# OnurBasci/TransformerBasedNavierStokeSolver

Measured on AMD Instinct MI355X. Metric: ns64_train_samples_per_s, higher is better.
Workload: dtype f32

## Files before the change

transformerbasednavierstokesolver_amd/csrc/pa2d_gemm.hip:

```cpp
#include "pa2d_gemm_common.h"
#include <string.h>


static Pa2dEnv read_env() {
    auto is = [](const char* n, const char* pre) { const char* e = getenv(n); return e && strncmp(e, pre, strlen(pre)) == 0; };
    auto num = [](const char* n, int dflt) { const char* e = getenv(n); return (e && e[0]) ? atoi(e) : dflt; };
    Pa2dEnv v;
    v.conv_halo = is("PA2D_CONV_HALO", "o") ? 0 : (is("PA2D_CONV_HALO", "f") ? 2 : 1);
    v.mc_big_off = is("PA2D_MC_BIG", "o") ? 1 : 0;
    v.kc_bk16 = num("PA2D_KC_BK", 0) == 16 ? 1 : 0;
    v.mc_bk = num("PA2D_MC_BK", 16) == 32 ? 32 : 16;
    v.mc_splits = num("PA2D_MC_SPLITS", 0);
    v.mcb_splits = num("PA2D_MCB_SPLITS", 0);
    v.lin_dw_split = is("PA2D_LIN_DW_SPLIT", "of") ? 0 : 1;
    v.lin_panel = is("PA2D_LIN_PANEL", "of") ? 0 : 1;
    v.lin_rowpanel = is("PA2D_LIN_ROWPANEL", "of") ? 0 : 1;
    v.lin_small_split = is("PA2D_LIN_SMALL_SPLIT", "of") ? 0 : 1;
    v.conv_mfma16 = num("PA2D_CONV_MFMA", 16) == 32 ? 0 : 1;
    v.split_big = num("PA2D_SPLIT_BIG", 1);
    v.slice_map = is("PA2D_SLICE_MAP", "l") ? 0 : 1;
    v.default_engine = is("PA2D_GEMM", "f") ? 0 : (is("PA2D_GEMM", "b") ? 2 : 1);
    return v;
}
static Pa2dEnv g_env = read_env();
const Pa2dEnv& pa2d_env() { return g_env; }
static int kc_bk(bool im2col, int Cin) {
    if (im2col && pa2d_env().kc_bk16) return 16;
    return (!im2col || (Cin % 32) == 0) ? 32 : 16;
}
KCTile kc_tile(int M, int N, bool im2col, int Cin) {
    const int tiles_m = ceil_div(M, 128);
    const long long t128 = (long long)tiles_m * ceil_div(N, 128);
    const long long t12864 = (long long)tiles_m * ceil_div(N, 64);
    const int bk = kc_bk(im2col, Cin);
    if (N > 64 && t128 >= 384) return {128, 128, bk};
    if (t12864 >= 384 || M <= 64) return {128, 64, bk};
    return {64, 64, bk};
}
bool use_split(int engine, int N, bool im2col, int Cin) {
    const int m = engine;
    if (m == 1) return im2col && N > 64 && (Cin % 32) == 0;
    if (m == 2) return N > 64 && (!im2col || (Cin % 32) == 0);
    return false;
}

int launch_kc(const KCParams& p_in, bool im2col, hipStream_t st, hipEvent_t ev0, hipEvent_t ev1) {
    KCParams p = p_in;
    if (!engine_ok(p.engine)) return PA2D_ERR_ARG;
    if (p.M <= 0 || p.N <= 0 || p.K <= 0) return PA2D_OK;
    if (!p.bias2) p.bias_split = 0x7fffffff;
    {
        const unsigned long long ab = ((unsigned long long)(p.M - 1) * p.lda + (im2col ? p.Cin : p.K)) * 4ull;
        const unsigned long long bb = ((unsigned long long)(p.N - 1) * p.ldb + p.K) * 4ull;
        if (ab >= 0xFFFFFFF0ull || bb >= 0xFFFFFFF0ull) return PA2D_ERR_UNSUPPORTED;
        p.a_bytes = (unsigned)ab;
        p.b_bytes = (unsigned)bb;
        const unsigned long long es = p.io_bf16 ? 2ull : 4ull;
        const unsigned long long cb = ((unsigned long long)(p.M - 1) * p.ldc + p.N) * es;
        const unsigned long long rb = p.res ? ((unsigned long long)(p.M - 1) * p.ldres + p.N) * es : 0ull;
        const unsigned long long xb = p.aux ? ((unsigned long long)(p.M - 1) * p.ldaux + p.N) * es : 0ull;
        if (cb >= 0xFFFFFFF0ull || rb >= 0xFFFFFFF0ull || xb >= 0xFFFFFFF0ull) return PA2D_ERR_UNSUPPORTED;
        p.c_bytes = (unsigned)cb; p.res_bytes = (unsigned)rb; p.aux_bytes = (unsigned)xb;
    }
    if ((p.K & 3) || (p.lda & 3) || (p.ldb & 3)) return PA2D_ERR_ARG;
    if (im2col && ((p.Cin & 15) || p.K != (p.taps == 27 ? 27 : 9) * p.Cin)) return PA2D_ERR_UNSUPPORTED;
    if (im2col && (p.epi != 0 || p.res)) return PA2D_ERR_ARG;
    if (ev0 && hipEventRecord(ev0, st) != hipSuccess) return PA2D_ERR_ARG;
    int rc;
    if (!im2col && p.wimg && rowpanel_applies(p)) {
        if (p.wsrc) {
            rc = launch_pack_weight_image(p.wsrc, p.wsn, p.wsk, p.wimg, p.N, p.K, st);
            if (rc) return rc;
        }
        KCParams pp = p;
        pp.M = p.M - p.M % 128;
        rc = launch_kc_rowpanel(pp, p.wimg, st);
        if (!rc && pp.M < p.M) {
            KCParams pt = p_in;
            pt.wimg = nullptr;
            pt.M = p.M - pp.M;
            pt.A = p.A + (size_t)pp.M * p.lda;
            pt.C = p.C + (size_t)pp.M * p.ldc;
            if (p.res) pt.res = p.res + (size_t)pp.M * p.ldres;
            if (p.aux) pt.aux = p.aux + (size_t)pp.M * p.ldaux;
            rc = launch_kc(pt, false, st);
        }
    } else if (panel_applies(p, im2col)) {
        KCParams pp = p;
        pp.M = p.M - p.M % 256;
        rc = launch_kc_panel(pp, st);
        if (!rc && pp.M < p.M) {
            KCParams pt = p_in;
            const size_t ea = p.io_bf16 ? 2 : 4, es = p.io_bf16 ? 2 : 4;
            pt.M = p.M - pp.M;
            pt.A = (const float*)((const char*)p.A + (size_t)pp.M * p.lda * ea);
            pt.C = (float*)((char*)p.C + (size_t)pp.M * p.ldc * es);
            if (p.res) pt.res = (const float*)((const char*)p.res + (size_t)pp.M * p.ldres * es);
            if (p.aux) pt.aux = (float*)((char*)p.aux + (size_t)pp.M * p.ldaux * es);
            rc = launch_kc(pt, false, st);
        }
    } else if (p.io_bf16 || use_split(p.engine, p.N, im2col, p.Cin)) rc = launch_kc_split(p, im2col, st);
    else if (kc_split_small_applies(p, im2col)) rc = launch_kc_split_small(p, st);
    else rc = launch_kc_f32(p, im2col, kc_tile(p.M, p.N, im2col, p.Cin), st);
    if (rc) return rc;
    if (ev1 && hipEventRecord(ev1, st) != hipSuccess) return PA2D_ERR_ARG;
    return PA2D_OK;
}

template <int TAPS>
__global__ void repack_kernel(const float* __restrict__ w0, const float* __restrict__ w1, float* __restrict__ dst,
                              int mode, int N, int K, int C, int Cin, int NK) {
    const long long idx = (long long)blockIdx.x * blockDim.x + threadIdx.x;
    if (mode == 0) {
        if (idx >= (long long)N * K) return;
        const int n = (int)(idx % N), k = (int)(idx / N);
        dst[idx] = w0[(size_t)n * K + k];
    } else if (mode == 1) {
        if (idx >= (long long)NK * C * TAPS * Cin) return;
        const int CH = K;
        const int c16 = (int)(idx % CH);
        const int tap = (int)((idx / CH) % TAPS);
        const int cic = (int)((idx / (TAPS * CH)) % (Cin / CH));
        const int co = (int)(idx / ((long long)Cin * TAPS));
        const int ci = cic * CH + c16;
        const float* src = co < C ? w0 : w1;
        dst[idx] = src[((size_t)(co % C) * Cin + ci) * TAPS + tap];
    } else {
        if (idx >= (long long)NK * C * TAPS * Cin) return;
        const int CH = K;
        const int c16 = (int)(idx % CH);
        const int tap = (int)((idx / CH) % TAPS);
        const int cic = (int)((idx / (TAPS * CH)) % (NK * C / CH));
        const int ci = (int)(idx / ((long long)NK * C * TAPS));
        const int co = cic * CH + c16;
        const float* src = co < C ? w0 : w1;
        dst[idx] = src[((size_t)(co % C) * Cin + ci) * TAPS + (TAPS - 1 - tap)];
    }
}

int launch_repack(const float* w0, const float* w1, float* dst, int mode, int N, int K, int C, int Cin, hipStream_t st,
                  int taps) {
    const int nk = w1 ? 2 : 1;
    const long long count = mode == 0 ? (long long)N * K : (long long)nk * C * taps * Cin;
    const dim3 grid((unsigned)ceil_div_ll(count, 256));
    if (taps == 27)
        hipLaunchKernelGGL(repack_kernel<27>, grid, dim3(256), 0, st, w0, w1, dst, mode, N, K, C, Cin, nk);
    else
        hipLaunchKernelGGL(repack_kernel<9>, grid, dim3(256), 0, st, w0, w1, dst, mode, N, K, C, Cin, nk);
    PA2D_CHECK_LAUNCH();
    return PA2D_OK;
}

static KCParams dense_fwd_params(const void* x, long long ldx, const float* w, long long ldw, const float* bias,
                                 const void* res, long long ldres, void* y, long long ldy, void* pre, long long ldpre, int M,
                                 int N, int K, int act, int engine, bool io_bf16) {
    KCParams p = {};
    p.engine = engine; p.io_bf16 = io_bf16 ? 1 : 0; p.apre = io_bf16 ? 1 : 0;
    p.aux_deriv = (act & PA2D_ACT_SAVE_DERIVATIVE_BIT) ? 1 : 0;
    act &= ~PA2D_ACT_SAVE_DERIVATIVE_BIT;
    p.A = (const float*)x; p.lda = ldx; p.B = w; p.ldb = ldw; p.C = (float*)y; p.ldc = ldy; p.bias = bias;
    p.res = (const float*)res; p.ldres = ldres; p.aux = (float*)pre; p.ldaux = ldpre; p.M = M; p.N = N; p.K = K; p.act = act;
    p.epi = (act != ACT_NONE ? EPI_ACT : 0) | (pre ? EPI_STORE_PRE : 0);
    return p;
}
static KCParams dense_bwd_data_params(const void* dy, long long lddy, const float* wt, const void* pre, long long ldpre,
                                      int act, void* dx, long long lddx, int M, int N, int K, int engine, bool io_bf16) {
// ... 133 lines not shown
```

transformerbasednavierstokesolver_amd/csrc/pa2d_gemm_mc_planes.hip:

```cpp
#include "pa2d_gemm_common.h"
#include "pa2d_bf16_split.h"

struct MCPlanesParams {
    const void* PA; int chA;
    const void* PB; int chB;
    float* slab;
    int Mi, Nj, Mk, chunks_per_split, splits, H, W, Cin;
    unsigned a_bytes, b_bytes;
    int taps;
    long long lda, ldb;
    float* colsum;
};

__device__ __forceinline__ unsigned img_off(int row, int ch) {
    return 256u * row + 16u * (ch ^ (((row & 3) << 2) | ((row >> 2) & 3)));
}

template <int NT, int KS, bool F32SRC = false>
__global__ __launch_bounds__(256, 2) void gemm_mc_planes_kernel(const MCPlanesParams p) {
    constexpr int PIMG = 4096;
    constexpr int STAGE = 2 * NT * KS * PIMG;
    constexpr int NP = 2 * NT * KS;
    __shared__ __attribute__((aligned(16))) unsigned char smem[2 * STAGE];

// ... 69 lines not shown
            bool ok_ = m_ < p.Mk && (KS == 1 || (c_) + (s_row[s] >> 4) < c_end);    \
            int mm_ = m_;                                                                                 \
            if (s_isb[s]) {                                                                               \
                const int n_ = m_ % HW;                                                                   \
                const int y_ = n_ / p.W, x_ = n_ - y_ * p.W;                                              \
                ok_ = ok_ && (unsigned)(y_ + tap_dy) < (unsigned)p.H && (unsigned)(x_ + tap_dx) < (unsigned)p.W; \
                mm_ = m_ + tap_shift;                                                                     \
            }                                                                                             \
            const unsigned rowb_ = (unsigned)mm_ * (unsigned)((s_isb[s] ? p.chB : p.chA) * NT * 64);      \
            rg[s] = s_isb[s] ? __builtin_amdgcn_raw_buffer_load_b128(rb_rsrc, ok_ ? rowb_ + s_goff[s] : OOB_OFF, 0, 0) \
                             : __builtin_amdgcn_raw_buffer_load_b128(ra_rsrc, ok_ ? rowb_ + s_goff[s] : OOB_OFF, 0, 0); \
        }                                                                                                 \
    }
#define MP_STORE(buf_)                                                                                    \
    if constexpr (F32SRC) {                                                                               \
        _Pragma("unroll") for (int ks = 0; ks < KS; ++ks) _Pragma("unroll") for (int op = 0; op < 2; ++op) { \
            const u32x4 u0_ = rg[ks * 4 + op * 2], u1_ = rg[ks * 4 + op * 2 + 1];                         \
            const float4 v0_ = make_float4(__uint_as_float(u0_.x), __uint_as_float(u0_.y), __uint_as_float(u0_.z), __uint_as_float(u0_.w)); \
            const float4 v1_ = make_float4(__uint_as_float(u1_.x), __uint_as_float(u1_.y), __uint_as_float(u1_.z), __uint_as_float(u1_.w)); \
            if (op == 0 && do_cs) {                                                                       \
                cs[0] += v0_.x; cs[1] += v0_.y; cs[2] += v0_.z; cs[3] += v0_.w;                           \
                cs[4] += v1_.x; cs[5] += v1_.y; cs[6] += v1_.z; cs[7] += v1_.w;                           \
            }                                                                                             \
            bf16x4 h0_, m0_, l0_, h1_, m1_, l1_;                                                          \
            split3(v0_, h0_, m0_, l0_);                                                                   \
            split3(v1_, h1_, m1_, l1_);                                                                   \
            unsigned char* d_ = smem + (buf_) * STAGE + flds;                                             \
            *reinterpret_cast<bf16x8*>(d_ + ((op * NT + 0) * KS + ks) * PIMG) = __builtin_shufflevector(h0_, h1_, 0, 1, 2, 3, 4, 5, 6, 7); \
            if (NT == 3) {                                                                                \
                *reinterpret_cast<bf16x8*>(d_ + ((op * NT + 1) * KS + ks) * PIMG) = __builtin_shufflevector(m0_, m1_, 0, 1, 2, 3, 4, 5, 6, 7); \
                *reinterpret_cast<bf16x8*>(d_ + ((op * NT + 2) * KS + ks) * PIMG) = __builtin_shufflevector(l0_, l1_, 0, 1, 2, 3, 4, 5, 6, 7); \
            }                                                                                             \
        }                                                                                                 \
    } else {                                                                                              \
        _Pragma("unroll") for (int s = 0; s < NP; ++s)                                                    \
            *reinterpret_cast<u32x4*>(smem + (buf_) * STAGE + s_lds[s]) = rg[s];                          \
    }
    const bool do_cs = F32SRC && p.colsum != nullptr && tj == 0;

    f32x16 acc[2][2];
#pragma unroll
    for (int i = 0; i < 2; ++i)
#pragma unroll
        for (int j = 0; j < 2; ++j)
#pragma unroll
            for (int r = 0; r < 16; ++r) acc[i][j][r] = 0.f;

    const int g = lane >> 4, q4 = (lane & 15) >> 2, pq = lane & 3;
    unsigned fa[2][2], fb[2][2];
#pragma unroll
    for (int t = 0; t < 2; ++t)
#pragma unroll
        for (int r = 0; r < 2; ++r) {
            const int row = 8 * (g >> 1) + 4 * r + q4;
            const int cha = ((wm * 64 + t * 32) >> 3) + 2 * (g & 1) + (pq >> 1);
            const int chb = ((wn * 64 + t * 32) >> 3) + 2 * (g & 1) + (pq >> 1);
            fa[t][r] = img_off(row, cha) + 8u * (pq & 1);
            fb[t][r] = img_off(row, chb) + 8u * (pq & 1);
        }

    if (c_begin < c_end) {
        MP_LOAD(c_begin)
        MP_STORE(0)
    }
    __syncthreads();
    for (int c = c_begin; c < c_end; c += KS) {
        const int buf = ((c - c_begin) / KS) & 1;
        if (c + KS < c_end) { MP_LOAD(c + KS) }
#pragma unroll
        for (int ks = 0; ks < KS; ++ks) {
        const unsigned char* st = smem + buf * STAGE + ks * PIMG;
        bf16x8 af[2][NT], bf[2][NT];
#pragma unroll
        for (int t = 0; t < 2; ++t)
#pragma unroll
            for (int pl = 0; pl < NT; ++pl) {
                typedef __attribute__((address_space(3))) s16x4 lds_s16x4;
                const s16x4 a0 = __builtin_amdgcn_ds_read_tr16_b64_v4i16((lds_s16x4*)(st + pl * KS * PIMG + fa[t][0]));
                const s16x4 a1 = __builtin_amdgcn_ds_read_tr16_b64_v4i16((lds_s16x4*)(st + pl * KS * PIMG + fa[t][1]));
                const s16x4 b0 = __builtin_amdgcn_ds_read_tr16_b64_v4i16((lds_s16x4*)(st + (NT + pl) * KS * PIMG + fb[t][0]));
                const s16x4 b1 = __builtin_amdgcn_ds_read_tr16_b64_v4i16((lds_s16x4*)(st + (NT + pl) * KS * PIMG + fb[t][1]));
                const s16x8 av = __builtin_shufflevector(a0, a1, 0, 1, 2, 3, 4, 5, 6, 7);
                const s16x8 bv = __builtin_shufflevector(b0, b1, 0, 1, 2, 3, 4, 5, 6, 7);
                af[t][pl] = __builtin_bit_cast(bf16x8, av);
                bf[t][pl] = __builtin_bit_cast(bf16x8, bv);
            }
#pragma unroll
        for (int i = 0; i < 2; ++i)
#pragma unroll
            for (int j = 0; j < 2; ++j) {
                if constexpr (NT == 3) {
                    acc[i][j] = __builtin_amdgcn_mfma_f32_32x32x16_bf16(af[i][1], bf[j][1], acc[i][j], 0, 0, 0);
                    acc[i][j] = __builtin_amdgcn_mfma_f32_32x32x16_bf16(af[i][2], bf[j][0], acc[i][j], 0, 0, 0);
                    acc[i][j] = __builtin_amdgcn_mfma_f32_32x32x16_bf16(af[i][0], bf[j][2], acc[i][j], 0, 0, 0);
                    acc[i][j] = __builtin_amdgcn_mfma_f32_32x32x16_bf16(af[i][1], bf[j][0], acc[i][j], 0, 0, 0);
                    acc[i][j] = __builtin_amdgcn_mfma_f32_32x32x16_bf16(af[i][0], bf[j][1], acc[i][j], 0, 0, 0);
                }
                acc[i][j] = __builtin_amdgcn_mfma_f32_32x32x16_bf16(af[i][0], bf[j][0], acc[i][j], 0, 0, 0);
            }
        }
        if (c + KS < c_end) { MP_STORE(buf ^ 1) }
        __syncthreads();
    }
#undef MP_LOAD
#undef MP_STORE

    if constexpr (F32SRC) {
        if (do_cs) {
            float* sm = reinterpret_cast<float*>(smem);
#pragma unroll
            for (int e = 0; e < 8; ++e) sm[frow * 128 + fc8 * 8 + e] = cs[e];
            __syncthreads();
            if (tid < 128) {
                float t = 0.f;
#pragma unroll
                for (int r = 0; r < 16; ++r) t += sm[r * 128 + tid];
                if (ti * 128 + tid < p.Mi) p.colsum[(size_t)split * p.Mi + ti * 128 + tid] = t;
            }
        }
    }
    float* out = p.slab + (size_t)split * p.Mi * p.Nj;
    const int col0 = tj * 128 + wn * 64 + (lane & 31);
    const int row0 = ti * 128 + wm * 64 + 4 * (lane >> 5);
#pragma unroll
    for (int j = 0; j < 2; ++j)
#pragma unroll
        for (int i = 0; i < 2; ++i)
#pragma unroll
            for (int r = 0; r < 16; ++r) {
                const int row = row0 + i * 32 + (r & 3) + 8 * (r >> 2);
                if (!F32SRC || (row < p.Mi && col0 + j * 32 < p.Nj)) out[(size_t)row * p.Nj + col0 + j * 32] = acc[i][j][r];
            }
}

bool mc_planes_supported(int C, int Cin) { return (C % 64) == 0 && (Cin % 128) == 0; }

int launch_mc_planes(const void* PA, const void* PB, int C, int Cin, int Mk, int H, int W, float* slab,
                     const MCPlan& pl, int NT, hipStream_t st) {
    if (!mc_planes_supported(C, Cin) || !pl.big) return PA2D_ERR_UNSUPPORTED;
    MCPlanesParams p;
    p.PA = PA; p.chA = 2 * C / 32; p.PB = PB; p.chB = Cin / 32; p.slab = slab;
    p.Mi = 2 * C; p.Nj = 9 * Cin; p.Mk = Mk; p.chunks_per_split = pl.chunks_per_split; p.splits = pl.splits;
    p.H = H; p.W = W; p.Cin = Cin; p.taps = 9;
    const unsigned long long ab = (unsigned long long)Mk * p.chA * NT * 64, bb = (unsigned long long)Mk * p.chB * NT * 64;
    if (ab >= 0xFFFFFFF0ull || bb >= 0xFFFFFFF0ull) return PA2D_ERR_UNSUPPORTED;
    p.a_bytes = (unsigned)ab; p.b_bytes = (unsigned)bb;
    const dim3 grid((p.Mi / 128) * (p.Nj / 128) * pl.splits);
    if (NT == 3) hipLaunchKernelGGL((gemm_mc_planes_kernel<3, 1>), grid, dim3(256), 0, st, p);
    else hipLaunchKernelGGL((gemm_mc_planes_kernel<1, 4>), grid, dim3(256), 0, st, p);
    PA2D_CHECK_LAUNCH();
    return PA2D_OK;
}

template <int NT, int KS>
__global__ __launch_bounds__(512, 1) void gemm_mc_planes_big_kernel(const MCPlanesParams p, const int per_xcd) {
    constexpr int PIMG = 8192;
    constexpr int STAGE = 2 * NT * KS * PIMG;
    constexpr int NP = (2 * NT * KS * 512) / 512;
    extern __shared__ __attribute__((aligned(16))) unsigned char smem[];

    const int tid = threadIdx.x, lane = tid & 63, wave = tid >> 6;
    const int tiles_i = (p.Mi + 255) / 256, tiles_j = (p.Nj + 255) / 256;
    const int tiles = tiles_i * tiles_j;
    const int lin = (blockIdx.x & 7) * per_xcd + (blockIdx.x >> 3);
    if ((int)(blockIdx.x >> 3) >= per_xcd || lin >= tiles * p.splits) return;
    const int split = lin / tiles, t_ = lin - split * tiles;
    const int ti = t_ / tiles_j, tj = t_ - ti * tiles_j;
    const int wm = wave >> 2, wn = wave & 3;
    const int total_chunks = (p.Mk + 15) / 16;
    const int c_begin = split * p.chunks_per_split;
    const int c_end = min(total_chunks, c_begin + p.chunks_per_split);
    const int HW = p.taps == 1 ? 1 : p.H * p.W;

    const __amdgpu_buffer_rsrc_t ra_rsrc = __builtin_amdgcn_make_buffer_rsrc(const_cast<void*>(p.PA), 0, p.a_bytes, 0x00020000);
    const __amdgpu_buffer_rsrc_t rb_rsrc = __builtin_amdgcn_make_buffer_rsrc(const_cast<void*>(p.PB), 0, p.b_bytes, 0x00020000);

    const int row16 = tid >> 5, cgrp = (tid & 31) >> 2, piece = tid & 3;
    const bool colok_a = ti * 256 + cgrp * 32 < p.Mi;
    const unsigned goff_a = (unsigned)((((ti * 256) >> 5) + cgrp) * NT * 64 + piece * 16);
    const int jc = tj * 256 + cgrp * 32;
    const int tap = p.taps == 1 ? 4 : jc / p.Cin;
    const bool colok_b = jc < p.Nj;
    const unsigned goff_b = (unsigned)((p.taps == 1 ? (jc >> 5) : ((jc - tap * p.Cin) >> 5)) * NT * 64 + piece * 16);
    const int tap_dy = tap / 3 - 1, tap_dx = tap - (tap / 3) * 3 - 1, tap_shift = tap_dy * p.W + tap_dx;
    const unsigned pitch_a = (unsigned)(p.chA * NT * 64), pitch_b = (unsigned)(p.chB * NT * 64);
    const unsigned lds_off = 512u * row16 + 16u * ((unsigned)(cgrp * 4 + piece) ^ (unsigned)(((row16 & 3) << 2) | ((row16 >> 2) & 3)));
#define MB_LOAD(c_, RG)                                                                                   \
    {                                                                                                     \
        _Pragma("unroll") for (int ks = 0; ks < KS; ++ks) {                                               \
            const int m_ = ((c_) + ks) * 16 + row16;                                                      \
            const bool okr_ = m_ < p.Mk && (c_) + ks < c_end;             \
            bool okb_ = okr_ && colok_b;                                                                  \
            int mm_ = m_;                                                                                 \
            if (p.taps != 1) {       \
                okb_ = okb_ && (unsigned)(ly + tap_dy) < (unsigned)p.H && (unsigned)(lx + tap_dx) < (unsigned)p.W; \
                mm_ = m_ + tap_shift;                                                                     \
                lx += 16;                                                                                 \
                while (lx >= p.W) { lx -= p.W; ++ly; }                                                    \
                while (ly >= p.H) ly -= p.H;                                                              \
            }                                                                                             \
            const unsigned oa_ = (okr_ && colok_a) ? (unsigned)m_ * pitch_a + goff_a : OOB_OFF;           \
            const unsigned ob_ = okb_ ? (unsigned)mm_ * pitch_b + goff_b : OOB_OFF;                       \
            _Pragma("unroll") for (int pl = 0; pl < NT; ++pl) {                                           \
                RG[pl * KS + ks] = __builtin_amdgcn_raw_buffer_load_b128(ra_rsrc, oa_ == OOB_OFF ? OOB_OFF : oa_ + pl * 64u, 0, 0); \
                RG[(NT + pl) * KS + ks] = __builtin_amdgcn_raw_buffer_load_b128(rb_rsrc, ob_ == OOB_OFF ? OOB_OFF : ob_ + pl * 64u, 0, 0); \
            }                                                                                             \
        }                                                                                                 \
    }
#define MB_STORE(buf_, RG)                                                                                \
    {                                                                                                     \
        _Pragma("unroll") for (int s = 0; s < NP; ++s)                                                    \
            *reinterpret_cast<u32x4*>(smem + (buf_) * STAGE + s * PIMG + lds_off) = RG[s];                \
    }
    u32x4 rg0[NP];
    int ly = 0, lx = 0;
    if (p.taps != 1) {
        const int n0 = (c_begin * 16 + row16) % HW;
        ly = n0 / p.W;
        lx = n0 - ly * p.W;
    }

    f32x16 acc[4][2];
#pragma unroll
    for (int i = 0; i < 4; ++i)
#pragma unroll
        for (int j = 0; j < 2; ++j)
#pragma unroll
            for (int r = 0; r < 16; ++r) acc[i][j][r] = 0.f;

    const int g = lane >> 4, q4 = (lane & 15) >> 2, pq = lane & 3;
    unsigned fa[4][2], fb[2][2];
#pragma unroll
    for (int r = 0; r < 2; ++r) {
        const int row = 8 * (g >> 1) + 4 * r + q4;
        const unsigned swz = (unsigned)(((row & 3) << 2) | ((row >> 2) & 3));
#pragma unroll
        for (int t = 0; t < 4; ++t) {
            const int cha = ((wm * 128 + t * 32) >> 3) + 2 * (g & 1) + (pq >> 1);
            fa[t][r] = 512u * row + 16u * ((unsigned)cha ^ swz) + 8u * (pq & 1);
        }
#pragma unroll
        for (int t = 0; t < 2; ++t) {
            const int chb = ((wn * 64 + t * 32) >> 3) + 2 * (g & 1) + (pq >> 1);
            fb[t][r] = 512u * row + 16u * ((unsigned)chb ^ swz) + 8u * (pq & 1);
        }
    }

#define MB_COMPUTE(buf_)                                                                                  \
    _Pragma("unroll") for (int ks = 0; ks < KS; ++ks) {                                                   \
        const unsigned char* st = smem + (buf_) * STAGE + ks * PIMG;                                      \
        bf16x8 af[4][NT], bf[2][NT];                                                                      \
        typedef __attribute__((address_space(3))) s16x4 lds_s16x4;                                        \
        _Pragma("unroll") for (int pl = 0; pl < NT; ++pl) {                                               \
            _Pragma("unroll") for (int t = 0; t < 4; ++t) {                                               \
                const s16x4 a0 = __builtin_amdgcn_ds_read_tr16_b64_v4i16((lds_s16x4*)(st + pl * KS * PIMG + fa[t][0])); \
                const s16x4 a1 = __builtin_amdgcn_ds_read_tr16_b64_v4i16((lds_s16x4*)(st + pl * KS * PIMG + fa[t][1])); \
                af[t][pl] = __builtin_bit_cast(bf16x8, __builtin_shufflevector(a0, a1, 0, 1, 2, 3, 4, 5, 6, 7)); \
            }                                                                                             \
            _Pragma("unroll") for (int t = 0; t < 2; ++t) {                                               \
                const s16x4 b0 = __builtin_amdgcn_ds_read_tr16_b64_v4i16((lds_s16x4*)(st + (NT + pl) * KS * PIMG + fb[t][0])); \
                const s16x4 b1 = __builtin_amdgcn_ds_read_tr16_b64_v4i16((lds_s16x4*)(st + (NT + pl) * KS * PIMG + fb[t][1])); \
                bf[t][pl] = __builtin_bit_cast(bf16x8, __builtin_shufflevector(b0, b1, 0, 1, 2, 3, 4, 5, 6, 7)); \
            }                                                                                             \
        }                                                                                                 \
        _Pragma("unroll") for (int i = 0; i < 4; ++i)                                                     \
            _Pragma("unroll") for (int j = 0; j < 2; ++j) {                                               \
                if constexpr (NT == 3) {                                        \
                    acc[i][j] = __builtin_amdgcn_mfma_f32_32x32x16_bf16(af[i][1], bf[j][1], acc[i][j], 0, 0, 0); \
                    acc[i][j] = __builtin_amdgcn_mfma_f32_32x32x16_bf16(af[i][2], bf[j][0], acc[i][j], 0, 0, 0); \
                    acc[i][j] = __builtin_amdgcn_mfma_f32_32x32x16_bf16(af[i][0], bf[j][2], acc[i][j], 0, 0, 0); \
                    acc[i][j] = __builtin_amdgcn_mfma_f32_32x32x16_bf16(af[i][1], bf[j][0], acc[i][j], 0, 0, 0); \
                    acc[i][j] = __builtin_amdgcn_mfma_f32_32x32x16_bf16(af[i][0], bf[j][1], acc[i][j], 0, 0, 0); \
                }                                                                                         \
                acc[i][j] = __builtin_amdgcn_mfma_f32_32x32x16_bf16(af[i][0], bf[j][0], acc[i][j], 0, 0, 0); \
            }                                                                                             \
    }
    if (c_begin < c_end) {
        MB_LOAD(c_begin, rg0)
        MB_STORE(0, rg0)
        if (c_begin + KS < c_end) MB_LOAD(c_begin + KS, rg0)
    }
    __syncthreads();
    for (int c = c_begin; c < c_end; c += KS) {
        const int buf = ((c - c_begin) / KS) & 1;
        if (c + KS < c_end) {
            MB_STORE(buf ^ 1, rg0)
            if (c + 2 * KS < c_end) MB_LOAD(c + 2 * KS, rg0)
        }
        MB_COMPUTE(buf)
        __syncthreads();
    }
#undef MB_COMPUTE
#undef MB_LOAD
#undef MB_STORE

    float* out = p.slab + (size_t)split * p.Mi * p.Nj;
    const int col0 = tj * 256 + wn * 64 + (lane & 31);
    const int row0 = ti * 256 + wm * 128 + 4 * (lane >> 5);
#pragma unroll
    for (int j = 0; j < 2; ++j) {
        const int col = col0 + j * 32;
        if (col >= p.Nj) continue;
#pragma unroll
        for (int i = 0; i < 4; ++i)
#pragma unroll
            for (int r = 0; r < 16; ++r) {
                const int row = row0 + i * 32 + (r & 3) + 8 * (r >> 2);
                if (row < p.Mi) out[(size_t)row * p.Nj + col] = acc[i][j][r];
            }
    }
}

MCPlan plan_mc_planes_big(int Mi, int Nj, int Mk) {
    MCPlan pl;
    if (Mk < 1) Mk = 1;
    pl.big = 2;
    const int tiles = ceil_div(Mi, 256) * ceil_div(Nj, 256);
    const int total_chunks = ceil_div(Mk, 16);
    int splits = 256 / tiles;
    if (pa2d_env().mcb_splits > 0) splits = pa2d_env().mcb_splits;
    const int max_splits = total_chunks / 8 > 0 ? total_chunks / 8 : 1;
    if (splits > max_splits) splits = max_splits;
    if (splits < 1) splits = 1;
    pl.chunks_per_split = ceil_div(total_chunks, splits);
    pl.splits = ceil_div(total_chunks, pl.chunks_per_split);
    pl.slab_floats = (size_t)pl.splits * Mi * Nj;
    return pl;
}

bool mc_planes_big_applies(int C, int Cin, int Mk) {
    if (pa2d_env().mc_big_off) return false;
    return (C % 16) == 0 && (Cin % 32) == 0 && 2 * C >= 256 && 9 * Cin >= 256 && Mk >= 16 * 8 * 4;
}

int launch_mc_planes_big(const void* PA, const void* PB, int C, int Cin, int Mk, int H, int W, float* slab,
                         const MCPlan& pl, int NT, hipStream_t st) {
    return launch_mc_planes_big_raw(PA, 2 * C, PB, Cin, 9, Mk, H, W, slab, pl, NT, st);
}

int launch_mc_planes_big_raw(const void* PA, int Mi, const void* PB, int Cin, int taps, int Mk, int H, int W, float* slab,
                             const MCPlan& pl, int NT, hipStream_t st) {
    if ((Mi & 31) || (Cin & 31) || (taps != 1 && taps != 9)) return PA2D_ERR_UNSUPPORTED;
    MCPlanesParams p;
    p.PA = PA; p.chA = Mi / 32; p.PB = PB; p.chB = Cin / 32; p.slab = slab;
    p.Mi = Mi; p.Nj = taps * Cin; p.Mk = Mk; p.chunks_per_split = pl.chunks_per_split; p.splits = pl.splits;
    p.H = H; p.W = W; p.Cin = Cin; p.taps = taps;
    const unsigned long long ab = (unsigned long long)Mk * p.chA * NT * 64, bb = (unsigned long long)Mk * p.chB * NT * 64;
    if (ab >= 0xFFFFFFF0ull || bb >= 0xFFFFFFF0ull) return PA2D_ERR_UNSUPPORTED;
    p.a_bytes = (unsigned)ab; p.b_bytes = (unsigned)bb;
    const int wgs = ceil_div(p.Mi, 256) * ceil_div(p.Nj, 256) * pl.splits;
    const int per_xcd = ceil_div(wgs, 8);
    const dim3 grid(per_xcd * 8);
    if (NT == 3) {
        const int smem = 2 * 2 * 3 * 1 * 8192;
        {
            hipError_t e = hipFuncSetAttribute(reinterpret_cast<const void*>(&gemm_mc_planes_big_kernel<3, 1>),
                                               hipFuncAttributeMaxDynamicSharedMemorySize, smem);
            if (e != hipSuccess) return (int)e;
        }
        hipLaunchKernelGGL((gemm_mc_planes_big_kernel<3, 1>), grid, dim3(512), smem, st, p, per_xcd);
    } else {
        const int smem = 2 * 2 * 1 * 4 * 8192;
        {
            hipError_t e = hipFuncSetAttribute(reinterpret_cast<const void*>(&gemm_mc_planes_big_kernel<1, 4>),
                                               hipFuncAttributeMaxDynamicSharedMemorySize, smem);
            if (e != hipSuccess) return (int)e;
        }
        hipLaunchKernelGGL((gemm_mc_planes_big_kernel<1, 4>), grid, dim3(512), smem, st, p, per_xcd);
    }
    PA2D_CHECK_LAUNCH();
    return PA2D_OK;
}

bool mc_f32src_applies(int Mi, int Nj, int Mk, long long lda, long long ldb) {
    return pa2d_env().lin_dw_split && (Mi % 8) == 0 && (Nj % 8) == 0 && Mi > 64 && Nj > 64 && Mk >= 16 * 8 * 16 && (lda % 4) == 0 && (ldb % 4) == 0;
}

int launch_mc_f32src(const float* A, long long lda, int Mi, const float* B, long long ldb, int Nj, int Mk, float* slab,
                     const MCPlan& pl, int NT, float* colsum, hipStream_t st) {
    if (!pl.big) return PA2D_ERR_UNSUPPORTED;
    MCPlanesParams p = {};
    p.PA = A; p.PB = B; p.slab = slab; p.lda = lda; p.ldb = ldb; p.colsum = colsum;
    p.Mi = Mi; p.Nj = Nj; p.Mk = Mk; p.chunks_per_split = pl.chunks_per_split; p.splits = pl.splits;
    p.H = 1; p.W = 1; p.Cin = Nj; p.taps = 1; p.chA = 0; p.chB = 0;
    const unsigned long long ab = ((unsigned long long)(Mk - 1) * lda + Mi) * 4ull, bb = ((unsigned long long)(Mk - 1) * ldb + Nj) * 4ull;
    if (ab >= 0xFFFFFFF0ull || bb >= 0xFFFFFFF0ull) return PA2D_ERR_UNSUPPORTED;
    p.a_bytes = (unsigned)ab; p.b_bytes = (unsigned)bb;
    const dim3 grid(ceil_div(Mi, 128) * ceil_div(Nj, 128) * pl.splits);
    if (NT == 3) hipLaunchKernelGGL((gemm_mc_planes_kernel<3, 1, true>), grid, dim3(256), 0, st, p);
    else hipLaunchKernelGGL((gemm_mc_planes_kernel<1, 4, true>), grid, dim3(256), 0, st, p);
    PA2D_CHECK_LAUNCH();
    return PA2D_OK;
}
```

transformerbasednavierstokesolver_amd/csrc/pa2d_internal.h:

```cpp
#pragma once
#include <hip/hip_runtime.h>
#include <stdint.h>

typedef float f32x16 __attribute__((ext_vector_type(16)));
typedef float f32x4 __attribute__((ext_vector_type(4)));

#define PA2D_OK 0
#define PA2D_ERR_ARG 1001
#define PA2D_ERR_UNSUPPORTED 1002
#define PA2D_ERR_WORKSPACE 1003

#define PA2D_CHECK_LAUNCH()                         \
    do {                                            \
        hipError_t e__ = hipGetLastError();         \
        if (e__ != hipSuccess) return (int)e__;     \
    } while (0)

enum { ACT_NONE = 0, ACT_GELU = 1, ACT_TANH = 2, ACT_SIGMOID = 3, ACT_RELU = 4, ACT_SOFTPLUS = 5,
       ACT_ELU = 6, ACT_SILU = 7 };

__device__ __forceinline__ float normal_cdf(float x, float& e_out) {
#pragma clang fp contract(off)
    const float z = fabsf(x) * 0.70710678118654752440f;
    const float t = __builtin_amdgcn_rcpf(fmaf(0.3275911f, z, 1.0f));
    float poly = fmaf(1.061405429f, t, -1.453152027f);
    poly = fmaf(poly, t, 1.421413741f);
    poly = fmaf(poly, t, -0.284496736f);
    poly = fmaf(poly, t, 0.254829592f);
    const float e = __builtin_amdgcn_exp2f(-z * z * 1.44269504088896340736f);
    e_out = e;
    const float hq = 0.5f * poly * t * e;
    return x < 0.f ? hq : 1.0f - hq;
}
__device__ __forceinline__ float gelu_exact(float x) {
#pragma clang fp contract(off)
    float e;
    return x * normal_cdf(x, e);
}
__device__ __forceinline__ float dgelu_exact(float x) {
#pragma clang fp contract(off)
    float e;
    const float cdf = normal_cdf(x, e);
    return fmaf(x * 0.39894228040143267794f, e, cdf);
}

__device__ __forceinline__ float act_fwd(int id, float x) {
    switch (id) {
        case ACT_GELU: return gelu_exact(x);
        case ACT_TANH: return tanhf(x);
        case ACT_SIGMOID: return 1.0f / (1.0f + expf(-x));
        case ACT_RELU: return x > 0.f ? x : 0.f;
        case ACT_SOFTPLUS: return x > 20.f ? x : log1pf(expf(x));
        case ACT_ELU: return x > 0.f ? x : expm1f(x);
        case ACT_SILU: return x / (1.0f + expf(-x));
        default: return x;
    }
}

__device__ __forceinline__ float act_bwd(int id, float x) {
    switch (id) {
        case ACT_GELU: return dgelu_exact(x);
        case ACT_TANH: { const float t = tanhf(x); return 1.0f - t * t; }
        case ACT_SIGMOID: { const float s = 1.0f / (1.0f + expf(-x)); return s * (1.0f - s); }
        case ACT_RELU: return x > 0.f ? 1.f : 0.f;
        case ACT_SOFTPLUS: return x > 20.f ? 1.f : 1.0f / (1.0f + expf(-x));
        case ACT_ELU: return x > 0.f ? 1.f : expf(x);
        case ACT_SILU: { const float s = 1.0f / (1.0f + expf(-x)); return s * (1.0f + x * (1.0f - s)); }
        default: return 1.f;
    }
}

__device__ __forceinline__ float wave_sum(float v) {
#pragma unroll
    for (int o = 32; o > 0; o >>= 1) v += __shfl_xor(v, o, 64);
    return v;
}
__device__ __forceinline__ float wave_max(float v) {
#pragma unroll
    for (int o = 32; o > 0; o >>= 1) v = fmaxf(v, __shfl_xor(v, o, 64));
    return v;
}

typedef unsigned int u32x4 __attribute__((ext_vector_type(4)));
#define OOB_OFF 0xFFFFFFFFu

__device__ __forceinline__ __amdgpu_buffer_rsrc_t make_rsrc(const float* base, unsigned bytes) {
    return __builtin_amdgcn_make_buffer_rsrc(const_cast<float*>(base), 0, bytes, 0x00020000);
}
__device__ __forceinline__ float4 buf_load4(__amdgpu_buffer_rsrc_t r, unsigned voff) {
    const u32x4 v = __builtin_amdgcn_raw_buffer_load_b128(r, voff, 0, 0);
    return make_float4(__uint_as_float(v.x), __uint_as_float(v.y), __uint_as_float(v.z), __uint_as_float(v.w));
}


__device__ __forceinline__ float buf_load1(__amdgpu_buffer_rsrc_t r, unsigned voff) {
    return __uint_as_float(__builtin_amdgcn_raw_buffer_load_b32(r, voff, 0, 0));
}
__device__ __forceinline__ void buf_store1(__amdgpu_buffer_rsrc_t r, unsigned voff, float v) {
    __builtin_amdgcn_raw_buffer_store_b32(__float_as_uint(v), r, voff, 0, 0);
}

__device__ __forceinline__ float2 buf_load2(__amdgpu_buffer_rsrc_t r, unsigned voff) {
    typedef unsigned int u32x2_ __attribute__((ext_vector_type(2)));
    const u32x2_ v = __builtin_amdgcn_raw_buffer_load_b64(r, voff, 0, 0);
    return make_float2(__uint_as_float(v.x), __uint_as_float(v.y));
}
__device__ __forceinline__ void buf_store4(__amdgpu_buffer_rsrc_t r, unsigned voff, float4 v) {
    u32x4 u = {__float_as_uint(v.x), __float_as_uint(v.y), __float_as_uint(v.z), __float_as_uint(v.w)};
    __builtin_amdgcn_raw_buffer_store_b128(u, r, voff, 0, 0);
}

#define PA2D_ACT_SAVE_DERIVATIVE_BIT 0x100

struct Pa2dEnv {
    int conv_halo;
    int mc_big_off;
    int kc_bk16;
    int mc_bk;
    int mc_splits;
    int mcb_splits;
    int lin_dw_split;
    int lin_panel;
    int conv_mfma16;
    int lin_small_split;
    int lin_rowpanel;
    int split_big;
    int slice_map;
    int default_engine;
};
const Pa2dEnv& pa2d_env();

static inline int pa2d_zero(void* p, size_t bytes, hipStream_t st) {
    if (!p || !bytes) return PA2D_OK;
    return (int)hipMemsetAsync(p, 0, bytes, st);
}
static inline int ceil_div(int a, int b) { return (a + b - 1) / b; }
static inline long long ceil_div_ll(long long a, long long b) { return (a + b - 1) / b; }

struct ReduceSegs { int nseg; long long begin[5]; float* dst[4]; };
int pa2d_launch_reduce_segs(const float* slab, int nslab, long long count, const ReduceSegs& segs, int accumulate,
                            hipStream_t st);

typedef __bf16 bf16_t;
template <typename T> struct Act;
template <> struct Act<float> {
    static constexpr unsigned ES = 4;
    static __device__ __forceinline__ float4 ld4(const float* p) { return *reinterpret_cast<const float4*>(p); }
    static __device__ __forceinline__ void st4(float* p, float4 v) { *reinterpret_cast<float4*>(p) = v; }
    static __device__ __forceinline__ float ld1(const float* p) { return *p; }
    static __device__ __forceinline__ float4 bld4(__amdgpu_buffer_rsrc_t r, unsigned off) { return buf_load4(r, off); }
    static __device__ __forceinline__ float2 bld2(__amdgpu_buffer_rsrc_t r, unsigned off) { return buf_load2(r, off); }
    static __device__ __forceinline__ float bld1(__amdgpu_buffer_rsrc_t r, unsigned off) { return buf_load1(r, off); }
    static __device__ __forceinline__ float bld1s(__amdgpu_buffer_rsrc_t r, unsigned off, unsigned soff) {
        return __uint_as_float(__builtin_amdgcn_raw_buffer_load_b32(r, off, soff, 0));
    }
    static __device__ __forceinline__ void bst4(__amdgpu_buffer_rsrc_t r, unsigned off, float4 v) { buf_store4(r, off, v); }
    static __device__ __forceinline__ void bst1(__amdgpu_buffer_rsrc_t r, unsigned off, float v) { buf_store1(r, off, v); }
};
__device__ __forceinline__ float bf16_bits_to_f32(unsigned short b) { return __uint_as_float((unsigned)b << 16); }
__device__ __forceinline__ unsigned short f32_to_bf16_bits(float x) {
    const bf16_t h = (bf16_t)x;
    return __builtin_bit_cast(unsigned short, h);
}
__device__ __forceinline__ unsigned pack_bf16x2(float lo, float hi) {
    return (unsigned)f32_to_bf16_bits(lo) | ((unsigned)f32_to_bf16_bits(hi) << 16);
}
template <> struct Act<bf16_t> {
    static constexpr unsigned ES = 2;
    static __device__ __forceinline__ float4 unpack4(uint2 q) {
        return make_float4(__uint_as_float(q.x << 16), __uint_as_float(q.x & 0xFFFF0000u), __uint_as_float(q.y << 16),
                           __uint_as_float(q.y & 0xFFFF0000u));
    }
    static __device__ __forceinline__ float4 ld4(const bf16_t* p) { return unpack4(*reinterpret_cast<const uint2*>(p)); }
    static __device__ __forceinline__ void st4(bf16_t* p, float4 v) {
        *reinterpret_cast<uint2*>(p) = make_uint2(pack_bf16x2(v.x, v.y), pack_bf16x2(v.z, v.w));
    }
    static __device__ __forceinline__ float ld1(const bf16_t* p) { return (float)*p; }
    static __device__ __forceinline__ float4 bld4(__amdgpu_buffer_rsrc_t r, unsigned off) {
        typedef unsigned int u32x2_ __attribute__((ext_vector_type(2)));
        const u32x2_ q = __builtin_amdgcn_raw_buffer_load_b64(r, off, 0, 0);
        return unpack4(make_uint2(q.x, q.y));
    }
    static __device__ __forceinline__ float2 bld2(__amdgpu_buffer_rsrc_t r, unsigned off) {
        const unsigned q = __builtin_amdgcn_raw_buffer_load_b32(r, off, 0, 0);
        return make_float2(__uint_as_float(q << 16), __uint_as_float(q & 0xFFFF0000u));
    }
    static __device__ __forceinline__ float bld1(__amdgpu_buffer_rsrc_t r, unsigned off) {
        return bf16_bits_to_f32(__builtin_amdgcn_raw_buffer_load_b16(r, off, 0, 0));
    }
    static __device__ __forceinline__ float bld1s(__amdgpu_buffer_rsrc_t r, unsigned off, unsigned soff) {
        return bf16_bits_to_f32(__builtin_amdgcn_raw_buffer_load_b16(r, off, soff, 0));
    }
    static __device__ __forceinline__ void bst4(__amdgpu_buffer_rsrc_t r, unsigned off, float4 v) {
        typedef unsigned int u32x2_ __attribute__((ext_vector_type(2)));
        const u32x2_ q = {pack_bf16x2(v.x, v.y), pack_bf16x2(v.z, v.w)};
        __builtin_amdgcn_raw_buffer_store_b64(q, r, off, 0, 0);
    }
    static __device__ __forceinline__ void bst1(__amdgpu_buffer_rsrc_t r, unsigned off, float v) {
        __builtin_amdgcn_raw_buffer_store_b16(f32_to_bf16_bits(v), r, off, 0, 0);
    }
};
__device__ __forceinline__ __amdgpu_buffer_rsrc_t make_rsrc_v(const void* base, unsigned bytes) {
    return __builtin_amdgcn_make_buffer_rsrc(const_cast<void*>(base), 0, bytes, 0x00020000);
}

__device__ __forceinline__ bool slice_decode(int xcd_map, int B, int heads, int nchunk, int& b, int& hh, int& chunk, int& bid) {
    const int total = B * heads * nchunk;
    int L;
    if (xcd_map) {
        const int per = (total + 7) >> 3;
        if ((int)(blockIdx.x >> 3) >= per) return false;
        L = (int)(blockIdx.x & 7) * per + (int)(blockIdx.x >> 3);
        if (L >= total) return false;
        hh = L % heads;
        chunk = (L / heads) % nchunk;
        b = L / (heads * nchunk);
    } else {
        L = (int)blockIdx.x;
        if (L >= total) return false;
        chunk = L % nchunk;
        hh = (L / nchunk) % heads;
        b = L / (nchunk * heads);
    }
    bid = (b * heads + hh) * nchunk + chunk;
    return true;
}
static inline int slice_grid(int total) { return ((total + 7) / 8) * 8; }
```

Measured before the change: 68.44.

## Stagger MFMA schedule across wave halves in big multi-chunk planes GEMM

Adds a staggered variant of the big planes GEMM kernel for the NT=3 case, on by default. Waves 4-7 defer most of their MFMAs for each K-step into the next iteration, running them before the next LDS store and global load. The aim is to shift half the workgroup out of phase so LDS reads, global loads and MFMA work overlap instead of every wave bursting in lockstep between barriers. The cost is extra live fragment registers across the barrier, plus sched_barrier hints that limit the compiler's own scheduling.

```diff
diff --git a/transformerbasednavierstokesolver_amd/csrc/pa2d_gemm.hip b/transformerbasednavierstokesolver_amd/csrc/pa2d_gemm.hip
--- a/transformerbasednavierstokesolver_amd/csrc/pa2d_gemm.hip
+++ b/transformerbasednavierstokesolver_amd/csrc/pa2d_gemm.hip
@@ -12,6 +12,7 @@
     v.mc_bk = num("PA2D_MC_BK", 16) == 32 ? 32 : 16;
     v.mc_splits = num("PA2D_MC_SPLITS", 0);
     v.mcb_splits = num("PA2D_MCB_SPLITS", 0);
+    v.mcb_stagger = is("PA2D_MCB_STAGGER", "of") ? 0 : 1;
     v.lin_dw_split = is("PA2D_LIN_DW_SPLIT", "of") ? 0 : 1;
     v.lin_panel = is("PA2D_LIN_PANEL", "of") ? 0 : 1;
     v.lin_rowpanel = is("PA2D_LIN_ROWPANEL", "of") ? 0 : 1;
diff --git a/transformerbasednavierstokesolver_amd/csrc/pa2d_gemm_mc_planes.hip b/transformerbasednavierstokesolver_amd/csrc/pa2d_gemm_mc_planes.hip
--- a/transformerbasednavierstokesolver_amd/csrc/pa2d_gemm_mc_planes.hip
+++ b/transformerbasednavierstokesolver_amd/csrc/pa2d_gemm_mc_planes.hip
@@ -245,8 +245,9 @@
     return PA2D_OK;
 }
 
-template <int NT, int KS>
+template <int NT, int KS, bool STAG = false>
 __global__ __launch_bounds__(512, 1) void gemm_mc_planes_big_kernel(const MCPlanesParams p, const int per_xcd) {
+    static_assert(!STAG || KS == 1, "the staggered schedule defers part of ONE K-step");
     constexpr int PIMG = 8192;
     constexpr int STAGE = 2 * NT * KS * PIMG;
     constexpr int NP = (2 * NT * KS * 512) / 512;
@@ -339,34 +340,38 @@
         }
     }
 
+    typedef __attribute__((address_space(3))) s16x4 lds_s16x4;
+#define MB_READS(st_, AF, BF)                                                                             \
+    _Pragma("unroll") for (int pl = 0; pl < NT; ++pl) {                                                   \
+        _Pragma("unroll") for (int t = 0; t < 4; ++t) {                                                   \
+            const s16x4 a0 = __builtin_amdgcn_ds_read_tr16_b64_v4i16((lds_s16x4*)((st_) + pl * KS * PIMG + fa[t][0])); \
+            const s16x4 a1 = __builtin_amdgcn_ds_read_tr16_b64_v4i16((lds_s16x4*)((st_) + pl * KS * PIMG + fa[t][1])); \
+            AF[t][pl] = __builtin_bit_cast(bf16x8, __builtin_shufflevector(a0, a1, 0, 1, 2, 3, 4, 5, 6, 7)); \
+        }                                                                                                 \
+        _Pragma("unroll") for (int t = 0; t < 2; ++t) {                                                   \
+            const s16x4 b0 = __builtin_amdgcn_ds_read_tr16_b64_v4i16((lds_s16x4*)((st_) + (NT + pl) * KS * PIMG + fb[t][0])); \
+            const s16x4 b1 = __builtin_amdgcn_ds_read_tr16_b64_v4i16((lds_s16x4*)((st_) + (NT + pl) * KS * PIMG + fb[t][1])); \
+            BF[t][pl] = __builtin_bit_cast(bf16x8, __builtin_shufflevector(b0, b1, 0, 1, 2, 3, 4, 5, 6, 7)); \
+        }                                                                                                 \
+    }
+#define MB_MFMAS(T0, T1, AF, BF)                                                                          \
+    _Pragma("unroll") for (int t = (T0); t < (T1); ++t) {                                                 \
+        const int i = t >> 1, j = t & 1;                                                                  \
+        if constexpr (NT == 3) {                                                \
+            acc[i][j] = __builtin_amdgcn_mfma_f32_32x32x16_bf16(AF[i][1], BF[j][1], acc[i][j], 0, 0, 0);  \
+            acc[i][j] = __builtin_amdgcn_mfma_f32_32x32x16_bf16(AF[i][2], BF[j][0], acc[i][j], 0, 0, 0);  \
+            acc[i][j] = __builtin_amdgcn_mfma_f32_32x32x16_bf16(AF[i][0], BF[j][2], acc[i][j], 0, 0, 0);  \
+            acc[i][j] = __builtin_amdgcn_mfma_f32_32x32x16_bf16(AF[i][1], BF[j][0], acc[i][j], 0, 0, 0);  \
+            acc[i][j] = __builtin_amdgcn_mfma_f32_32x32x16_bf16(AF[i][0], BF[j][1], acc[i][j], 0, 0, 0);  \
+        }                                                                                                 \
+        acc[i][j] = __builtin_amdgcn_mfma_f32_32x32x16_bf16(AF[i][0], BF[j][0], acc[i][j], 0, 0, 0);      \
+    }
 #define MB_COMPUTE(buf_)                                                                                  \
     _Pragma("unroll") for (int ks = 0; ks < KS; ++ks) {                                                   \
         const unsigned char* st = smem + (buf_) * STAGE + ks * PIMG;                                      \
         bf16x8 af[4][NT], bf[2][NT];                                                                      \
-        typedef __attribute__((address_space(3))) s16x4 lds_s16x4;                                        \
-        _Pragma("unroll") for (int pl = 0; pl < NT; ++pl) {                                               \
-            _Pragma("unroll") for (int t = 0; t < 4; ++t) {                                               \
-                const s16x4 a0 = __builtin_amdgcn_ds_read_tr16_b64_v4i16((lds_s16x4*)(st + pl * KS * PIMG + fa[t][0])); \
-                const s16x4 a1 = __builtin_amdgcn_ds_read_tr16_b64_v4i16((lds_s16x4*)(st + pl * KS * PIMG + fa[t][1])); \
-                af[t][pl] = __builtin_bit_cast(bf16x8, __builtin_shufflevector(a0, a1, 0, 1, 2, 3, 4, 5, 6, 7)); \
-            }                                                                                             \
-            _Pragma("unroll") for (int t = 0; t < 2; ++t) {                                               \
-                const s16x4 b0 = __builtin_amdgcn_ds_read_tr16_b64_v4i16((lds_s16x4*)(st + (NT + pl) * KS * PIMG + fb[t][0])); \
-                const s16x4 b1 = __builtin_amdgcn_ds_read_tr16_b64_v4i16((lds_s16x4*)(st + (NT + pl) * KS * PIMG + fb[t][1])); \
-                bf[t][pl] = __builtin_bit_cast(bf16x8, __builtin_shufflevector(b0, b1, 0, 1, 2, 3, 4, 5, 6, 7)); \
-            }                                                                                             \
-        }                                                                                                 \
-        _Pragma("unroll") for (int i = 0; i < 4; ++i)                                                     \
-            _Pragma("unroll") for (int j = 0; j < 2; ++j) {                                               \
-                if constexpr (NT == 3) {                                        \
-                    acc[i][j] = __builtin_amdgcn_mfma_f32_32x32x16_bf16(af[i][1], bf[j][1], acc[i][j], 0, 0, 0); \
-                    acc[i][j] = __builtin_amdgcn_mfma_f32_32x32x16_bf16(af[i][2], bf[j][0], acc[i][j], 0, 0, 0); \
-                    acc[i][j] = __builtin_amdgcn_mfma_f32_32x32x16_bf16(af[i][0], bf[j][2], acc[i][j], 0, 0, 0); \
-                    acc[i][j] = __builtin_amdgcn_mfma_f32_32x32x16_bf16(af[i][1], bf[j][0], acc[i][j], 0, 0, 0); \
-                    acc[i][j] = __builtin_amdgcn_mfma_f32_32x32x16_bf16(af[i][0], bf[j][1], acc[i][j], 0, 0, 0); \
-                }                                                                                         \
-                acc[i][j] = __builtin_amdgcn_mfma_f32_32x32x16_bf16(af[i][0], bf[j][0], acc[i][j], 0, 0, 0); \
-            }                                                                                             \
+        MB_READS(st, af, bf)                                                                              \
+        MB_MFMAS(0, 8, af, bf)                                                                            \
     }
     if (c_begin < c_end) {
         MB_LOAD(c_begin, rg0)
@@ -374,16 +379,42 @@
         if (c_begin + KS < c_end) MB_LOAD(c_begin + KS, rg0)
     }
     __syncthreads();
-    for (int c = c_begin; c < c_end; c += KS) {
-        const int buf = ((c - c_begin) / KS) & 1;
-        if (c + KS < c_end) {
-            MB_STORE(buf ^ 1, rg0)
-            if (c + 2 * KS < c_end) MB_LOAD(c + 2 * KS, rg0)
-        }
-        MB_COMPUTE(buf)
-        __syncthreads();
+    constexpr int DEFER_FROM = 2;
+    bool delayed = false;
+    if constexpr (STAG) delayed = __builtin_amdgcn_readfirstlane(wave) >= 4;
+    if constexpr (STAG) {
+        if (delayed) {
+            bf16x8 af[4][NT], bf[2][NT];
+            for (int c = c_begin; c < c_end; ++c) {
+                const int buf = (c - c_begin) & 1;
+                if (c > c_begin) { MB_MFMAS(DEFER_FROM, 8, af, bf) }
+                __builtin_amdgcn_sched_barrier(0);
+                if (c + 1 < c_end) {
+                    MB_STORE(buf ^ 1, rg0)
+                    if (c + 2 < c_end) MB_LOAD(c + 2, rg0)
+                }
+                MB_READS(smem + buf * STAGE, af, bf)
+                MB_MFMAS(0, DEFER_FROM, af, bf)
+                __builtin_amdgcn_sched_barrier(0);
+                __syncthreads();
+            }
+            if (c_begin < c_end) { MB_MFMAS(DEFER_FROM, 8, af, bf) }
+        }
+    }
+    if (!delayed) {
+        for (int c = c_begin; c < c_end; c += KS) {
+            const int buf = ((c - c_begin) / KS) & 1;
+            if (c + KS < c_end) {
+                MB_STORE(buf ^ 1, rg0)
+                if (c + 2 * KS < c_end) MB_LOAD(c + 2 * KS, rg0)
+            }
+            MB_COMPUTE(buf)
+            __syncthreads();
+        }
     }
 #undef MB_COMPUTE
+#undef MB_MFMAS
+#undef MB_READS
 #undef MB_LOAD
 #undef MB_STORE
 
@@ -446,12 +477,15 @@
     const dim3 grid(per_xcd * 8);
     if (NT == 3) {
         const int smem = 2 * 2 * 3 * 1 * 8192;
+        const bool stag = pa2d_env().mcb_stagger != 0;
         {
-            hipError_t e = hipFuncSetAttribute(reinterpret_cast<const void*>(&gemm_mc_planes_big_kernel<3, 1>),
-                                               hipFuncAttributeMaxDynamicSharedMemorySize, smem);
+            const void* fn = stag ? reinterpret_cast<const void*>(&gemm_mc_planes_big_kernel<3, 1, true>)
+                                  : reinterpret_cast<const void*>(&gemm_mc_planes_big_kernel<3, 1, false>);
+            hipError_t e = hipFuncSetAttribute(fn, hipFuncAttributeMaxDynamicSharedMemorySize, smem);
             if (e != hipSuccess) return (int)e;
         }
-        hipLaunchKernelGGL((gemm_mc_planes_big_kernel<3, 1>), grid, dim3(512), smem, st, p, per_xcd);
+        if (stag) hipLaunchKernelGGL((gemm_mc_planes_big_kernel<3, 1, true>), grid, dim3(512), smem, st, p, per_xcd);
+        else hipLaunchKernelGGL((gemm_mc_planes_big_kernel<3, 1, false>), grid, dim3(512), smem, st, p, per_xcd);
     } else {
         const int smem = 2 * 2 * 1 * 4 * 8192;
         {
diff --git a/transformerbasednavierstokesolver_amd/csrc/pa2d_internal.h b/transformerbasednavierstokesolver_amd/csrc/pa2d_internal.h
--- a/transformerbasednavierstokesolver_amd/csrc/pa2d_internal.h
+++ b/transformerbasednavierstokesolver_amd/csrc/pa2d_internal.h
@@ -119,6 +119,7 @@
     int mc_bk;
     int mc_splits;
     int mcb_splits;
+    int mcb_stagger;
     int lin_dw_split;
     int lin_panel;
     int conv_mfma16;
```

Result: no change. 69.07, median of 6 (+0.9%).
